# 0xPARC/plonkathon

Hardware: NVIDIA H100
Metric: plonk_proofs_per_s_2^20_gates (higher is better)
Workload: dtype u256 (BN254 Fr/Fq integers, 8x32-bit Montgomery limbs)

## Files before the change

plonkathon_b200/csrc/host_selftest.cpp:

```cpp
#include "field.cuh"
#include "curve.cuh"
#include "msm_digits.cuh"
#include "modinv.cuh"
#include "msm_bucket.cuh"
#include "msm_sort.cuh"
#include "ntt_shard.cuh"
#include <algorithm>
#include <vector>
#include <cstring>
using namespace pb200;

template <class F> static F ld(const uint32_t* p) { F r; memcpy(r.v, p, 32); return r; }
template <class F> static void st(uint32_t* p, const F& a) { memcpy(p, a.v, 32); }

extern "C" {
int hs_field_op(int field, int op, const uint32_t* a, const uint32_t* b, uint32_t* out) {
#define RUN(F)                                                   \
  {                                                              \
    F x = ld<F>(a), y = ld<F>(b), r;                             \
    switch (op) {                                                \
      case 0: r = fp_add(x, y); break;                           \
      case 1: r = fp_sub(x, y); break;                           \
      case 2: r = fp_mul(x, y); break;                           \
      case 3: r = fp_neg(x); break;                              \
// ... 190 lines not shown
  g.batch = batch;
  g.own_log = 0;
  g.own_rank = 0;
  if (hi >= 0xfffffff0u && hi != 0xffffffffu) {
    g.own_log = 0xffffffffu - hi;
    g.own_rank = lo;
    g.lo = 0;
    g.nloc = g.half >> g.own_log;
    if (!g.nloc || lo >= (1u << g.own_log)) return false;
  } else {
    if (hi > g.half) hi = g.half;
    if (lo >= hi) return false;
    g.lo = lo;
    g.nloc = hi - lo;
  }
  g.sets = fixed_base ? batch : g.W;
  g.nb = g.sets * g.nloc;
  return true;
}

static void host_scan(uint32_t* cnt, uint32_t len, uint32_t pad, uint32_t* off, uint32_t* max_out) {
  uint32_t run = 0, m = 0;
  for (uint32_t b = 0; b < len; b++) {
    off[b] = run;
    run += (cnt[b] + pad) & ~pad;
    m = std::max(m, cnt[b]);
    cnt[b] = 0;
  }
  off[len] = run;
  if (max_out) *max_out = m;
}

static void host_msm_sort(const MsmGeom& g, const std::vector<Fr>& sc, uint32_t n, uint32_t pad, uint32_t lb,
                          uint32_t T, uint32_t spb, uint32_t bin_nt, uint32_t chunk_nt, std::vector<uint32_t>& counts,
                          std::vector<uint32_t>& off, std::vector<uint32_t>& sorted) {
  const uint32_t nbins = ((g.nb - 1) >> lb) + 1;
  const uint32_t batch = g.fixed_base ? g.batch : 1;
  std::vector<uint32_t> bin_cnt(nbins, 0), bin_off(nbins + 1), chunk_first(nbins + 1);
  std::vector<SortEntry> binned((size_t)n * g.W * batch);
  counts.assign(g.nb + 1, 0);
  off.assign(g.nb + 1, 0);
  SortArgs a;
  for (uint32_t k = 0; k < 4; k++) a.sb.p[k] = k < batch ? sc.data() + (size_t)k * n : nullptr;
  a.n = n;
  a.from_mont = 0;
  a.g = g;
  a.lb = lb;
  a.nbins = nbins;
  a.T = T;
  a.bin_cnt = bin_cnt.data();
  a.bin_off = bin_off.data();
  a.binned = binned.data();
  a.chunk_first = chunk_first.data();
  a.counts = counts.data();
  a.offsets = off.data();
  a.sorted = nullptr;
  a.spb = spb;
  std::vector<uint32_t> sh_cnt(std::max(nbins, 1u << lb)), sh_loc(sh_cnt.size()), sh_base(sh_cnt.size()), runs;
  std::vector<SortEntry> bin_stage_buf((size_t)spb * g.W);
  std::vector<uint32_t> chunk_stage_buf(T);
  auto block_scan = [&](uint32_t len, uint32_t nt) {
    runs.assign(nt, 0);
    uint32_t run = 0;
    for (uint32_t t = 0; t < nt; t++) { runs[t] = run; run += scan_part_sum(sh_cnt.data(), len, t, nt); }
    return run;
  };
  const uint32_t bin_blocks = (n + spb - 1) / spb;
  for (uint32_t k = 0; k < batch; k++)
    for (uint32_t bx = 0; bx < bin_blocks; bx++) {
      for (uint32_t t = 0; t < bin_nt; t++) sort_zero(sh_cnt.data(), nbins, t, bin_nt);
      for (uint32_t t = 0; t < bin_nt; t++) bin_hist(a, bx, k, t, bin_nt, sh_cnt.data());
      for (uint32_t t = 0; t < bin_nt; t++) bin_flush(a, t, bin_nt, sh_cnt.data());
    }
  host_scan(bin_cnt.data(), nbins, 0, bin_off.data(), nullptr);
  for (uint32_t k = batch; k-- > 0;)
    for (uint32_t bx = bin_blocks; bx-- > 0;) {
      for (uint32_t t = 0; t < bin_nt; t++) sort_zero(sh_cnt.data(), nbins, t, bin_nt);
      for (uint32_t t = 0; t < bin_nt; t++) bin_hist(a, bx, k, t, bin_nt, sh_cnt.data());
      const uint32_t total = block_scan(nbins, bin_nt);
      for (uint32_t t = 0; t < bin_nt; t++)
        bin_reserve(a, t, bin_nt, runs[t], sh_cnt.data(), sh_loc.data(), sh_base.data());
      for (uint32_t t = 0; t < bin_nt; t++) bin_stage(a, bx, k, t, bin_nt, sh_cnt.data(), sh_loc.data(), bin_stage_buf.data());
      for (uint32_t t = 0; t < bin_nt; t++)
        bin_copy_out(a, t, bin_nt, total, sh_loc.data(), sh_base.data(), bin_stage_buf.data());
    }
  {
    std::vector<uint32_t> sums(256);
    for (uint32_t t = 0; t < 256; t++) sums[t] = chunk_map_sum(a, t);
    uint32_t run = 0;
    for (uint32_t t = 0; t < 256; t++) { const uint32_t s = sums[t]; sums[t] = run; run += s; }
    for (uint32_t t = 0; t < 256; t++) chunk_map_write(a, t, sums[t], run);
  }
  const uint32_t grid = 3;
  SortChunk ch;
  for (uint32_t bx = 0; bx < grid; bx++)
    for (uint32_t c = bx; chunk_locate(a, c, ch); c += grid) {
      for (uint32_t t = 0; t < chunk_nt; t++) sort_zero(sh_cnt.data(), ch.nkeys, t, chunk_nt);
      for (uint32_t t = 0; t < chunk_nt; t++) chunk_hist(a, ch, t, chunk_nt, sh_cnt.data());
      for (uint32_t t = 0; t < chunk_nt; t++) chunk_flush(a, ch, t, chunk_nt, sh_cnt.data());
    }
  host_scan(counts.data(), g.nb, pad, off.data(), &counts[g.nb]);
  sorted.assign(off[g.nb] + 2, PB_MSM_PAD);
  a.sorted = sorted.data();
  for (uint32_t bx = grid; bx-- > 0;)
    for (uint32_t c = bx; chunk_locate(a, c, ch); c += grid) {
      for (uint32_t t = 0; t < chunk_nt; t++) sort_zero(sh_cnt.data(), ch.nkeys, t, chunk_nt);
      for (uint32_t t = 0; t < chunk_nt; t++) chunk_hist(a, ch, t, chunk_nt, sh_cnt.data());
      const uint32_t total = block_scan(ch.nkeys, chunk_nt);
      for (uint32_t t = 0; t < chunk_nt; t++)
        chunk_reserve(a, ch, t, chunk_nt, runs[t], sh_cnt.data(), sh_loc.data(), sh_base.data());
      for (uint32_t t = 0; t < chunk_nt; t++) chunk_stage(a, ch, t, chunk_nt, sh_cnt.data(), sh_loc.data(), chunk_stage_buf.data());
      for (uint32_t t = 0; t < chunk_nt; t++)
        chunk_copy_out(a, ch, t, chunk_nt, sh_loc.data(), sh_base.data(), chunk_stage_buf.data());
      if (total != ch.hi - ch.lo) abort();
    }
}

extern "C" {
int hs_msm_sort(const uint32_t* scalars, uint32_t n, uint32_t batch, uint32_t c, int fixed_base, uint32_t lo,
                uint32_t hi, uint32_t pad, uint32_t lb, uint32_t T, uint32_t spb, uint32_t bin_nt, uint32_t chunk_nt,
                uint32_t* counts_out, uint32_t* off_out, uint32_t* sorted_out, uint32_t cap) {
  if (!n || !batch || batch > 4 || (!fixed_base && batch != 1) || c < 1 || c > 16 || !T || !bin_nt || !chunk_nt)
    return -1;
  MsmGeom g;
  if (!msm_geom(n, batch, c, fixed_base, lo, hi, g)) return -1;
  if (lb == 0xffffffffu) lb = sort_default_lb(g.nb);
  if (((g.nb - 1) >> lb) >= PB_SORT_MAX_BINS || (1u << lb) > PB_SORT_MAX_BIN_KEYS) return -1;
  if (!spb) spb = PB_SORT_BIN_STAGE / g.W;
  std::vector<Fr> sc((size_t)batch * n);
  for (size_t i = 0; i < sc.size(); i++) sc[i] = ld<Fr>(scalars + 8 * i);
  std::vector<uint32_t> counts, off, sorted;
  host_msm_sort(g, sc, n, pad ? 1 : 0, lb, T, spb, bin_nt, chunk_nt, counts, off, sorted);
  if (off[g.nb] > cap) return -1;
  memcpy(counts_out, counts.data(), counts.size() * 4);
  memcpy(off_out, off.data(), off.size() * 4);
  memcpy(sorted_out, sorted.data(), (size_t)off[g.nb] * 4);
  return (int)g.nb;
}

int hs_msm_pipeline(const uint32_t* points, uint32_t n, const uint32_t* scalars, uint32_t batch, uint32_t c,
                    int fixed_base, uint32_t lo, uint32_t hi, uint32_t B, uint32_t g0, uint32_t* out, uint8_t* out_inf) {
  if (!n || !batch || batch > 4 || (!fixed_base && batch != 1) || c < 1 || c > 16 || B < 2 || B > PB_AFF_BMAX) return -1;
  if (g0 < 2 || (g0 & (g0 - 1))) return -1;
  MsmGeom g;
  if (!msm_geom(n, batch, c, fixed_base, lo, hi, g)) return -1;
  std::vector<G1Affine> tab(fixed_base ? (size_t)g.W * n : n);
  for (uint32_t i = 0; i < n; i++) {
    tab[i].x = fp_to_mont(ld<Fq>(points + 16 * i));
    tab[i].y = fp_to_mont(ld<Fq>(points + 16 * i + 8));
  }
  if (fixed_base)
    for (uint32_t w = 1; w < g.W; w++)
      for (uint32_t i = 0; i < n; i++) {
        G1XYZZ a;
        g1_double_affine(a, tab[(size_t)(w - 1) * n + i]);
        for (uint32_t k = 1; k < c; k++) g1_double(a);
        g1_to_affine(a, tab[(size_t)w * n + i]);
      }
  std::vector<Fr> sc((size_t)batch * n);
  for (size_t i = 0; i < sc.size(); i++) sc[i] = ld<Fr>(scalars + 8 * i);
  std::vector<uint32_t> counts, off, sorted;
  host_msm_sort(g, sc, n, 1, sort_default_lb(g.nb), PB_SORT_CHUNK, PB_SORT_BIN_STAGE / g.W, PB_SORT_BIN_THREADS,
                PB_SORT_CHUNK_THREADS, counts, off, sorted);
  const uint32_t maxc = counts[g.nb];
  const uint64_t positions = (uint64_t)n * g.W * batch + g.nb, s_bound = positions / 2;
  std::vector<G1Affine> pts(s_bound + 1);
  AffAcc a;
  a.table = tab.data();
  a.sorted = sorted.data();
  a.pts = pts.data();
  a.off = off.data();
  a.cnt = counts.data();
  a.max_cnt = counts.data() + g.nb;
  a.nbl = g.nb;
  a.B = B;
  Fq pref[PB_AFF_BMAX];
  uint32_t desc[PB_AFF_BMAX];
  int rounds = 0;
  for (uint32_t r = 0; r < 32; r++) {
    a.r = r;
    if (r > 0 && maxc > (1u << r)) rounds = r + 1;
    if (r == 0) rounds = 1;
    const uint64_t T = aff_round_threads(s_bound, B, r) + 40;
    for (uint64_t t = T; t-- > 0;) {
      if (r == 0) aff_round0_thread(a, t, pref, desc);
      else aff_round_thread(a, t, pref, desc);
    }
  }
  ReduceArgs ra;
  ra.pts = pts.data(); ra.off = off.data(); ra.cnt = counts.data(); ra.xb = nullptr;
  ra.sets = g.sets; ra.m = g.nloc; ra.g = g0;
  std::vector<SR> cur((size_t)g.sets * reduce_groups(ra.m, ra.g)), nxt;
  ra.out = cur.data();
  for (uint64_t t = 0; t < cur.size() + 3; t++) reduce_level0_thread(ra, t);
  uint32_t m = reduce_groups(ra.m, ra.g), log_G = 0;
  while ((1u << log_G) < g0) log_G++;
// ... 72 lines not shown
```

plonkathon_b200/csrc/msm.cu:

```cuda
#include <algorithm>
#include <cstring>

#include "common.cuh"
#include "comm.cuh"
#include "msm_bucket.cuh"
#include "msm_digits.cuh"
#include "msm_sort.cuh"

namespace pb200 {

__device__ __forceinline__ G1Affine ld_affine(const G1Affine* p) {
  const uint4* q = reinterpret_cast<const uint4*>(p);
  uint4 a = __ldg(q), b = __ldg(q + 1), c = __ldg(q + 2), d = __ldg(q + 3);
  G1Affine r;
  r.x.v[0] = a.x; r.x.v[1] = a.y; r.x.v[2] = a.z; r.x.v[3] = a.w;
  r.x.v[4] = b.x; r.x.v[5] = b.y; r.x.v[6] = b.z; r.x.v[7] = b.w;
  r.y.v[0] = c.x; r.y.v[1] = c.y; r.y.v[2] = c.z; r.y.v[3] = c.w;
  r.y.v[4] = d.x; r.y.v[5] = d.y; r.y.v[6] = d.z; r.y.v[7] = d.w;
  return r;
}

__device__ __forceinline__ uint32_t block_exclusive_scan(uint32_t v, uint32_t* sh, uint32_t* total) {
  const uint32_t lane = threadIdx.x & 31, wid = threadIdx.x >> 5, nw = blockDim.x >> 5;
  uint32_t x = v;
  for (int d = 1; d < 32; d <<= 1) {
    uint32_t y = __shfl_up_sync(0xffffffffu, x, d);
    if ((int)lane >= d) x += y;
  }
  if (lane == 31) sh[wid] = x;
  __syncthreads();
  if (wid == 0) {
    uint32_t w = lane < nw ? sh[lane] : 0;
    for (int d = 1; d < 32; d <<= 1) {
      uint32_t y = __shfl_up_sync(0xffffffffu, w, d);
      if ((int)lane >= d) w += y;
    }
    if (lane < nw) sh[lane] = w;
  }
  __syncthreads();
  uint32_t base = wid ? sh[wid - 1] : 0;
  *total = sh[nw - 1];
  __syncthreads();
  return base + x - v;
}

__global__ void __launch_bounds__(PB_SORT_BIN_THREADS) k_msm_bin_count(SortArgs a) {
  __shared__ uint32_t sh_cnt[PB_SORT_MAX_BINS];
  const uint32_t t = threadIdx.x, nt = blockDim.x;
  sort_zero(sh_cnt, a.nbins, t, nt);
  __syncthreads();
  bin_hist(a, blockIdx.x, blockIdx.y, t, nt, sh_cnt);
  __syncthreads();
  bin_flush(a, t, nt, sh_cnt);
}

__global__ void __launch_bounds__(PB_SORT_BIN_THREADS) k_msm_bin_scatter(SortArgs a) {
  __shared__ uint32_t sh_cnt[PB_SORT_MAX_BINS], sh_loc[PB_SORT_MAX_BINS], sh_base[PB_SORT_MAX_BINS], sh_scan[32];
  extern __shared__ SortEntry stage[];
  const uint32_t t = threadIdx.x, nt = blockDim.x;
  sort_zero(sh_cnt, a.nbins, t, nt);
  __syncthreads();
  bin_hist(a, blockIdx.x, blockIdx.y, t, nt, sh_cnt);
  __syncthreads();
  uint32_t total;
  const uint32_t run = block_exclusive_scan(scan_part_sum(sh_cnt, a.nbins, t, nt), sh_scan, &total);
  bin_reserve(a, t, nt, run, sh_cnt, sh_loc, sh_base);
  __syncthreads();
  bin_stage(a, blockIdx.x, blockIdx.y, t, nt, sh_cnt, sh_loc, stage);
  __syncthreads();
  bin_copy_out(a, t, nt, total, sh_loc, sh_base, stage);
}

__global__ void __launch_bounds__(PB_SORT_CHUNK_THREADS) k_msm_chunk_count(SortArgs a) {
  __shared__ uint32_t sh_cnt[PB_SORT_MAX_BIN_KEYS];
  const uint32_t t = threadIdx.x, nt = blockDim.x;
  SortChunk ch;
  for (uint32_t c = blockIdx.x; chunk_locate(a, c, ch); c += gridDim.x) {
    sort_zero(sh_cnt, ch.nkeys, t, nt);
    __syncthreads();
    chunk_hist(a, ch, t, nt, sh_cnt);
    __syncthreads();
    chunk_flush(a, ch, t, nt, sh_cnt);
    __syncthreads();
  }
}

__global__ void __launch_bounds__(PB_SORT_CHUNK_THREADS) k_msm_chunk_place(SortArgs a) {
  __shared__ uint32_t sh_cnt[PB_SORT_MAX_BIN_KEYS], sh_loc[PB_SORT_MAX_BIN_KEYS], sh_base[PB_SORT_MAX_BIN_KEYS],
      sh_scan[32];
  extern __shared__ uint32_t stage_vals[];
  const uint32_t t = threadIdx.x, nt = blockDim.x;
  SortChunk ch;
  for (uint32_t c = blockIdx.x; chunk_locate(a, c, ch); c += gridDim.x) {
    sort_zero(sh_cnt, ch.nkeys, t, nt);
    __syncthreads();
    chunk_hist(a, ch, t, nt, sh_cnt);
    __syncthreads();
    uint32_t total;
    const uint32_t run = block_exclusive_scan(scan_part_sum(sh_cnt, ch.nkeys, t, nt), sh_scan, &total);
    chunk_reserve(a, ch, t, nt, run, sh_cnt, sh_loc, sh_base);
    __syncthreads();
    chunk_stage(a, ch, t, nt, sh_cnt, sh_loc, stage_vals);
    __syncthreads();
// ... 452 lines not shown
    }
  } else {
    comm = nullptr;
  }
  if (bucket_hi > g.half) bucket_hi = g.half;
  PB_CHECK(bucket_lo < bucket_hi, "empty MSM bucket range");
  g.lo = bucket_lo;
  g.nloc = bucket_hi - bucket_lo;
  g.sets = fixed_base ? batch : g.W;
  g.nb = g.sets * g.nloc;
  PB_CHECK((fixed_base ? (uint64_t)g.W * point_stride : n) < (1ull << 31), "MSM too large for 31-bit point ids");
  ScalarBatch sb;
  for (uint32_t k = 0; k < 4; k++) sb.p[k] = k < batch ? scalars[k] : nullptr;

  static const bool use_xyzz = [] { const char* e = getenv("PB200_MSM_ACC"); return !(e && !strcmp(e, "affine")); }();
  const uint32_t pad = use_xyzz ? 0 : 1;
  DevBuf& sorted = ctx->scratch[2];
  DevBuf& counts = ctx->scratch[3];
  DevBuf& offsets = ctx->scratch[4];
  DevBuf& lvl_a = ctx->scratch[6];
  DevBuf& lvl_b = ctx->scratch[7];
  const uint64_t entries = n * g.W * batch;
  const uint64_t positions = entries + (pad ? g.nb : 0);
  PB_CHECK(positions < (1ull << 30), "MSM too large (n * windows * batch must stay below 2^30)");
  sorted.ensure(positions * 4);
  counts.ensure((size_t)g.nb * 4 + 16);
  offsets.ensure((size_t)(g.nb + 1) * 4);
  uint32_t* max_cnt = counts.as<uint32_t>() + g.nb;
  const uint32_t n_tiles = (g.nb + PB_SCAN_TILE - 1) / PB_SCAN_TILE;
  PB_CHECK(n_tiles <= 8192, "too many buckets for the scan");
  ctx->msm_aff[1].ensure((size_t)8192 * 4);
  uint32_t* tile_sums = ctx->msm_aff[1].as<uint32_t>();

  const uint32_t lb = sort_default_lb(g.nb);
  PB_CHECK((1u << lb) <= PB_SORT_MAX_BIN_KEYS, "too many buckets for the sort");
  DevBuf& binned = ctx->scratch[8];
  DevBuf& bin_tab = ctx->scratch[9];
  binned.ensure(entries * sizeof(SortEntry));
  bin_tab.ensure((size_t)3 * (PB_SORT_MAX_BINS + 1) * 4);
  SortArgs sa;
  sa.sb = sb;
  sa.n = n;
  sa.from_mont = scalars_mont ? 1 : 0;
  sa.g = g;
  sa.lb = lb;
  sa.nbins = ((g.nb - 1) >> lb) + 1;
  sa.T = PB_SORT_CHUNK;
  uint32_t* bin_cnt = bin_tab.as<uint32_t>();
  uint32_t* bin_off = bin_cnt + PB_SORT_MAX_BINS + 1;
  sa.bin_cnt = bin_cnt;
  sa.bin_off = bin_off;
  sa.binned = binned.as<SortEntry>();
  sa.chunk_first = bin_off + PB_SORT_MAX_BINS + 1;
  sa.counts = counts.as<uint32_t>();
  sa.offsets = offsets.as<uint32_t>();
  sa.sorted = sorted.as<uint32_t>();
  sa.spb = PB_SORT_BIN_STAGE / g.W;
  const dim3 bin_grid((unsigned)((n + sa.spb - 1) / sa.spb), batch);
  const uint64_t chunk_bound = entries / PB_SORT_CHUNK + sa.nbins;
  const uint32_t count_grid = (uint32_t)std::min<uint64_t>((uint64_t)ctx->sm_count * 4, chunk_bound);
  const uint32_t place_grid = (uint32_t)std::min<uint64_t>((uint64_t)ctx->sm_count * 2, chunk_bound);
  const size_t bin_stage_bytes = PB_SORT_BIN_STAGE * sizeof(SortEntry), chunk_stage_bytes = PB_SORT_CHUNK * 4;
  PB_CUDA(cudaFuncSetAttribute(k_msm_bin_scatter, cudaFuncAttributeMaxDynamicSharedMemorySize, (int)bin_stage_bytes));
  PB_CUDA(cudaFuncSetAttribute(k_msm_chunk_place, cudaFuncAttributeMaxDynamicSharedMemorySize, (int)chunk_stage_bytes));

  cudaStream_t st = ctx->stream;
  ctx->time_begin(2);
  PB_CUDA(cudaMemsetAsync(counts.p, 0, (size_t)g.nb * 4 + 16, st));
  PB_CUDA(cudaMemsetAsync(bin_cnt, 0, (size_t)sa.nbins * 4, st));
  if (pad) PB_CUDA(cudaMemsetAsync(sorted.p, 0xff, positions * 4, st));
  k_msm_bin_count<<<bin_grid, PB_SORT_BIN_THREADS, 0, st>>>(sa);
  k_scan_tile_sums<<<1, 256, 0, st>>>(bin_cnt, sa.nbins, 0, tile_sums, nullptr);
  k_scan_tiles<<<1, 256, 0, st>>>(tile_sums, 1, bin_off + sa.nbins);
  k_scan_apply<<<1, 256, 0, st>>>(bin_cnt, sa.nbins, 0, tile_sums, bin_off);
  k_msm_bin_scatter<<<bin_grid, PB_SORT_BIN_THREADS, bin_stage_bytes, st>>>(sa);
  k_msm_chunk_map<<<1, 256, 0, st>>>(sa);
  k_msm_chunk_count<<<count_grid, PB_SORT_CHUNK_THREADS, 0, st>>>(sa);
  k_scan_tile_sums<<<n_tiles, 256, 0, st>>>(counts.as<uint32_t>(), g.nb, pad, tile_sums, max_cnt);
  k_scan_tiles<<<1, 256, 0, st>>>(tile_sums, n_tiles, offsets.as<uint32_t>() + g.nb);
  k_scan_apply<<<n_tiles, 256, 0, st>>>(counts.as<uint32_t>(), g.nb, pad, tile_sums, offsets.as<uint32_t>());
  k_msm_chunk_place<<<place_grid, PB_SORT_CHUNK_THREADS, chunk_stage_bytes, st>>>(sa);
  ctx->time_end(2);
  ctx->launches += 11;

  ReduceArgs ra;
  ra.pts = nullptr; ra.off = offsets.as<uint32_t>(); ra.cnt = counts.as<uint32_t>(); ra.xb = nullptr;
  if (!use_xyzz) {
    const uint64_t s_bound = positions / 2;
    DevBuf& pts = ctx->msm_aff[0];
    pts.ensure(s_bound * sizeof(G1Affine));
    AffAcc a;
    a.table = points;
    a.sorted = sorted.as<uint32_t>();
    a.pts = pts.as<G1Affine>();
    a.off = offsets.as<uint32_t>();
    a.cnt = counts.as<uint32_t>();
    a.max_cnt = max_cnt;
    a.nbl = g.nb;
    uint64_t cap = fixed_base ? n * g.W : n;
    uint32_t max_rounds = 1;
    while (max_rounds < 32 && (1ull << max_rounds) < cap) max_rounds++;
    ctx->time_begin(0);
    for (uint32_t r = 0; r < std::min<uint32_t>(max_rounds, PB_AFF_GRID_ROUNDS); r++) {
      a.r = r;
      a.B = pick_B(ctx, s_bound, r);
      const uint64_t threads = aff_round_threads(s_bound, a.B, r);
      if (r == 0) k_aff_round0<<<(unsigned)((threads + 127) / 128), 128, 0, st>>>(a);
      else k_aff_round<<<(unsigned)((threads + 127) / 128), 128, 0, st>>>(a);
      ctx->launches++;
    }
    if (max_rounds > PB_AFF_GRID_ROUNDS) {
      a.B = 32;
      k_aff_tail<<<1, 256, 0, st>>>(a, s_bound);
      ctx->launches++;
    }
    ctx->time_end(0);
// ... 311 lines not shown
```

plonkathon_b200/csrc/msm_sort.cuh:

```cuda
#pragma once
#include "msm_digits.cuh"

namespace pb200 {

#define PB_SORT_MAX_BINS 2048
#define PB_SORT_MAX_BIN_KEYS 2048
#define PB_SORT_BIN_THREADS 512
#define PB_SORT_BIN_STAGE 8192
#define PB_SORT_CHUNK_THREADS 512
#define PB_SORT_CHUNK 16384
static_assert(PB_SORT_MAX_BINS <= 256 * 8, "k_msm_chunk_map and the bin scan take one block of 256 x 8 bins");

struct alignas(8) SortEntry {
  uint32_t key, val;
};

struct SortArgs {
  ScalarBatch sb;
  uint64_t n;
  int from_mont;
  MsmGeom g;
  uint32_t spb;
  uint32_t lb;
  uint32_t nbins;
  uint32_t T;
  uint32_t* bin_cnt;
  const uint32_t* bin_off;
  SortEntry* binned;
  uint32_t* chunk_first;
  uint32_t* counts;
  const uint32_t* offsets;
  uint32_t* sorted;
};

PB_HD uint32_t sort_default_lb(uint32_t nb) {
  uint32_t lb = 0;
  while (((nb - 1) >> lb) >= PB_SORT_MAX_BINS) lb++;
  return lb;
}

PB_HD uint32_t sort_add(uint32_t* p, uint32_t v) {
#if defined(__CUDA_ARCH__)
  return atomicAdd(p, v);
#else
  const uint32_t o = *p;
  *p = o + v;
  return o;
#endif
}

PB_HD void sort_zero(uint32_t* sh, uint32_t len, uint32_t t, uint32_t nt) {
  for (uint32_t b = t; b < len; b += nt) sh[b] = 0;
}

PB_HD uint32_t scan_part_sum(const uint32_t* sh, uint32_t len, uint32_t t, uint32_t nt) {
  const uint32_t per = (len + nt - 1) / nt;
  uint32_t s = 0;
  for (uint32_t b = t * per; b < t * per + per && b < len; b++) s += sh[b];
  return s;
}

template <class F>
PB_HD void sort_walk(const SortArgs& a, uint32_t bx, uint32_t k, uint32_t t, uint32_t nt, F f) {
  const uint64_t end = (uint64_t)(bx + 1) * a.spb < a.n ? (uint64_t)(bx + 1) * a.spb : a.n;
  for (uint64_t i = (uint64_t)bx * a.spb + t; i < end; i += nt) {
    DigitWalk dw(a.sb.p[k], i, a.from_mont);
    for (uint32_t w = 0; w < a.g.W; w++) {
      uint32_t neg, d = dw.next(w, a.g, neg);
      if (!d) continue;
      const uint32_t key = msm_bucket_key(a.g, k, w, d);
      if (key != 0xffffffffu) f(key, (uint32_t)((uint64_t)w * a.g.point_stride + i) | (neg << 31));
    }
  }
}

PB_HD void bin_hist(const SortArgs& a, uint32_t bx, uint32_t k, uint32_t t, uint32_t nt, uint32_t* sh_cnt) {
  sort_walk(a, bx, k, t, nt, [&](uint32_t key, uint32_t) { sort_add(&sh_cnt[key >> a.lb], 1u); });
}

PB_HD void bin_flush(const SortArgs& a, uint32_t t, uint32_t nt, const uint32_t* sh_cnt) {
  for (uint32_t b = t; b < a.nbins; b += nt)
    if (sh_cnt[b]) sort_add(&a.bin_cnt[b], sh_cnt[b]);
}

PB_HD void bin_reserve(const SortArgs& a, uint32_t t, uint32_t nt, uint32_t run, uint32_t* sh_cnt, uint32_t* sh_loc,
                       uint32_t* sh_base) {
  const uint32_t per = (a.nbins + nt - 1) / nt;
  for (uint32_t b = t * per; b < t * per + per && b < a.nbins; b++) {
    const uint32_t c = sh_cnt[b];
    sh_loc[b] = run;
    run += c;
    if (c) sh_base[b] = a.bin_off[b] + sort_add(&a.bin_cnt[b], c);
    sh_cnt[b] = 0;
  }
}

PB_HD void bin_stage(const SortArgs& a, uint32_t bx, uint32_t k, uint32_t t, uint32_t nt, uint32_t* sh_cnt,
                     const uint32_t* sh_loc, SortEntry* stage) {
  sort_walk(a, bx, k, t, nt, [&](uint32_t key, uint32_t val) {
    const uint32_t b = key >> a.lb;
    SortEntry e;
    e.key = key;
    e.val = val;
    stage[sh_loc[b] + sort_add(&sh_cnt[b], 1u)] = e;
  });
}

PB_HD void bin_copy_out(const SortArgs& a, uint32_t t, uint32_t nt, uint32_t total, const uint32_t* sh_loc,
                        const uint32_t* sh_base, const SortEntry* stage) {
  for (uint32_t p = t; p < total; p += nt) {
    const SortEntry e = stage[p];
    const uint32_t b = e.key >> a.lb;
    a.binned[sh_base[b] + p - sh_loc[b]] = e;
  }
}

PB_HD uint32_t chunk_map_sum(const SortArgs& a, uint32_t t) {
  uint32_t s = 0;
  for (uint32_t b = 8 * t; b < 8 * t + 8 && b < a.nbins; b++) s += (a.bin_cnt[b] + a.T - 1) / a.T;
  return s;
}
PB_HD void chunk_map_write(const SortArgs& a, uint32_t t, uint32_t run, uint32_t total) {
  for (uint32_t b = 8 * t; b < 8 * t + 8 && b < a.nbins; b++) {
    a.chunk_first[b] = run;
    run += (a.bin_cnt[b] + a.T - 1) / a.T;
  }
  if (t == 0) a.chunk_first[a.nbins] = total;
}

struct SortChunk {
  uint32_t lo, hi;
  uint32_t key0, nkeys;
};

PB_HD bool chunk_locate(const SortArgs& a, uint32_t c, SortChunk& ch) {
  if (c >= a.chunk_first[a.nbins]) return false;
  uint32_t l = 0, h = a.nbins;
  while (l < h) {
    const uint32_t m = (l + h) >> 1;
    if (a.chunk_first[m] > c) h = m; else l = m + 1;
  }
  const uint32_t b = l - 1;
  ch.lo = a.bin_off[b] + (c - a.chunk_first[b]) * a.T;
  ch.hi = a.bin_off[b + 1] - ch.lo > a.T ? ch.lo + a.T : a.bin_off[b + 1];
  ch.key0 = b << a.lb;
  ch.nkeys = a.g.nb - ch.key0 < (1u << a.lb) ? a.g.nb - ch.key0 : 1u << a.lb;
  return true;
}

PB_HD void chunk_hist(const SortArgs& a, const SortChunk& ch, uint32_t t, uint32_t nt, uint32_t* sh_cnt) {
  for (uint32_t i = ch.lo + t; i < ch.hi; i += nt) sort_add(&sh_cnt[a.binned[i].key - ch.key0], 1u);
}

PB_HD void chunk_flush(const SortArgs& a, const SortChunk& ch, uint32_t t, uint32_t nt, const uint32_t* sh_cnt) {
  for (uint32_t l = t; l < ch.nkeys; l += nt)
    if (sh_cnt[l]) sort_add(&a.counts[ch.key0 + l], sh_cnt[l]);
}

PB_HD void chunk_reserve(const SortArgs& a, const SortChunk& ch, uint32_t t, uint32_t nt, uint32_t run,
                         uint32_t* sh_cnt, uint32_t* sh_loc, uint32_t* sh_base) {
// ... 33 lines not shown
```

Before: 24.60.

## Add single-pass per-bin placement sort for MSM buckets with heavy-bin fallback

Adds a k_msm_bin_place kernel that, for bins small enough to fit in shared memory, counts, scans and scatters entries within one block, writing counts, offsets and sorted output directly. Bins above the cap take the old chunked path, with a new per-bin heavy scan replacing the global bucket-count scan when no padding is needed. Bin histograms are also limited to a per-batch window, bin-scan tiling is widened to multiple blocks, and the bin-width heuristic now targets the placement stage size. The aim is to remove the separate global count/scan/place passes and the large memsets. The cost is more code paths and a dependence on how the scalar distribution spreads across bins.

```diff
diff --git a/plonkathon_b200/csrc/host_selftest.cpp b/plonkathon_b200/csrc/host_selftest.cpp
--- a/plonkathon_b200/csrc/host_selftest.cpp
+++ b/plonkathon_b200/csrc/host_selftest.cpp
@@ -246,14 +246,18 @@
 }
 
 static void host_msm_sort(const MsmGeom& g, const std::vector<Fr>& sc, uint32_t n, uint32_t pad, uint32_t lb,
-                          uint32_t T, uint32_t spb, uint32_t bin_nt, uint32_t chunk_nt, std::vector<uint32_t>& counts,
-                          std::vector<uint32_t>& off, std::vector<uint32_t>& sorted) {
+                          uint32_t T, uint32_t spb, uint32_t bin_nt, uint32_t chunk_nt, uint32_t cap, uint32_t place_nt,
+                          std::vector<uint32_t>& counts, std::vector<uint32_t>& off, std::vector<uint32_t>& sorted,
+                          uint32_t* heavy = nullptr) {
   const uint32_t nbins = ((g.nb - 1) >> lb) + 1;
   const uint32_t batch = g.fixed_base ? g.batch : 1;
+  if (pad) cap = 0;
   std::vector<uint32_t> bin_cnt(nbins, 0), bin_off(nbins + 1), chunk_first(nbins + 1);
   std::vector<SortEntry> binned((size_t)n * g.W * batch);
-  counts.assign(g.nb + 1, 0);
-  off.assign(g.nb + 1, 0);
+  counts.assign(g.nb + 1, pad ? 0 : 0xdeadbeefu);
+  counts[g.nb] = 0;
+  off.assign(g.nb + 1, 0xdeadbeefu);
+  sorted.assign((size_t)n * g.W * batch + g.nb + 2, PB_MSM_PAD);
   SortArgs a;
   for (uint32_t k = 0; k < 4; k++) a.sb.p[k] = k < batch ? sc.data() + (size_t)k * n : nullptr;
   a.n = n;
@@ -262,42 +266,73 @@
   a.lb = lb;
   a.nbins = nbins;
   a.T = T;
+  a.cap = cap;
   a.bin_cnt = bin_cnt.data();
   a.bin_off = bin_off.data();
   a.binned = binned.data();
   a.chunk_first = chunk_first.data();
   a.counts = counts.data();
   a.offsets = off.data();
-  a.sorted = nullptr;
+  a.sorted = sorted.data();
   a.spb = spb;
   std::vector<uint32_t> sh_cnt(std::max(nbins, 1u << lb)), sh_loc(sh_cnt.size()), sh_base(sh_cnt.size()), runs;
   std::vector<SortEntry> bin_stage_buf((size_t)spb * g.W);
-  std::vector<uint32_t> chunk_stage_buf(T);
-  auto block_scan = [&](uint32_t len, uint32_t nt) {
+  std::vector<uint32_t> chunk_stage_buf(T), place_stage_buf(std::max(cap, 1u));
+  std::vector<uint32_t> kr((size_t)place_nt * PB_SORT_PLACE_PER), val(kr.size());
+  auto block_scan_of = [&](uint32_t nt, auto part) {
     runs.assign(nt, 0);
     uint32_t run = 0;
-    for (uint32_t t = 0; t < nt; t++) { runs[t] = run; run += scan_part_sum(sh_cnt.data(), len, t, nt); }
+    for (uint32_t t = 0; t < nt; t++) { runs[t] = run; run += part(t); }
     return run;
+  };
+  auto block_scan = [&](uint32_t len, uint32_t nt) {
+    return block_scan_of(nt, [&](uint32_t t) { return scan_part_sum(sh_cnt.data(), len, t, nt); });
   };
   const uint32_t bin_blocks = (n + spb - 1) / spb;
   for (uint32_t k = 0; k < batch; k++)
     for (uint32_t bx = 0; bx < bin_blocks; bx++) {
-      for (uint32_t t = 0; t < bin_nt; t++) sort_zero(sh_cnt.data(), nbins, t, bin_nt);
+      const uint32_t len = sort_window(g, lb, k).len;
+      for (uint32_t t = 0; t < bin_nt; t++) sort_zero(sh_cnt.data(), len, t, bin_nt);
       for (uint32_t t = 0; t < bin_nt; t++) bin_hist(a, bx, k, t, bin_nt, sh_cnt.data());
-      for (uint32_t t = 0; t < bin_nt; t++) bin_flush(a, t, bin_nt, sh_cnt.data());
+      for (uint32_t t = 0; t < bin_nt; t++) bin_flush(a, k, t, bin_nt, sh_cnt.data());
     }
   host_scan(bin_cnt.data(), nbins, 0, bin_off.data(), nullptr);
   for (uint32_t k = batch; k-- > 0;)
     for (uint32_t bx = bin_blocks; bx-- > 0;) {
-      for (uint32_t t = 0; t < bin_nt; t++) sort_zero(sh_cnt.data(), nbins, t, bin_nt);
+      const uint32_t len = sort_window(g, lb, k).len;
+      for (uint32_t t = 0; t < bin_nt; t++) sort_zero(sh_cnt.data(), len, t, bin_nt);
       for (uint32_t t = 0; t < bin_nt; t++) bin_hist(a, bx, k, t, bin_nt, sh_cnt.data());
-      const uint32_t total = block_scan(nbins, bin_nt);
+      const uint32_t total = block_scan(len, bin_nt);
       for (uint32_t t = 0; t < bin_nt; t++)
-        bin_reserve(a, t, bin_nt, runs[t], sh_cnt.data(), sh_loc.data(), sh_base.data());
+        bin_reserve(a, k, t, bin_nt, runs[t], sh_cnt.data(), sh_loc.data(), sh_base.data());
       for (uint32_t t = 0; t < bin_nt; t++) bin_stage(a, bx, k, t, bin_nt, sh_cnt.data(), sh_loc.data(), bin_stage_buf.data());
       for (uint32_t t = 0; t < bin_nt; t++)
-        bin_copy_out(a, t, bin_nt, total, sh_loc.data(), sh_base.data(), bin_stage_buf.data());
-    }
+        bin_copy_out(a, k, t, bin_nt, total, sh_loc.data(), sh_base.data(), bin_stage_buf.data());
+    }
+  if (!pad) {
+    if (heavy) *heavy = 0;
+    for (uint32_t b = nbins; b-- > 0;) {
+      const SortBin sb = sort_bin(a, b);
+      bool take = true;
+      for (uint32_t t = 0; t < place_nt; t++) take = place_begin(a, sb, b, t, place_nt);
+      if (!take) {
+        if (heavy) ++*heavy;
+        continue;
+      }
+      for (uint32_t t = 0; t < place_nt; t++) sort_zero(sh_cnt.data(), sb.nkeys, t, place_nt);
+      for (uint32_t t = 0; t < place_nt; t++)
+        place_load(a, sb, t, place_nt, sh_cnt.data(), kr.data() + t * PB_SORT_PLACE_PER, val.data() + t * PB_SORT_PLACE_PER);
+      const uint32_t total = block_scan(sb.nkeys, place_nt);
+      if (total != sb.hi - sb.lo) abort();
+      uint32_t m = 0;
+      for (uint32_t t = 0; t < place_nt; t++) m = std::max(m, place_offsets(a, sb, t, place_nt, runs[t], sh_cnt.data()));
+      for (uint32_t t = 0; t < place_nt; t++)
+        place_stage(sb, t, place_nt, sh_cnt.data(), kr.data() + t * PB_SORT_PLACE_PER, val.data() + t * PB_SORT_PLACE_PER,
+                    place_stage_buf.data());
+      counts[g.nb] = std::max(counts[g.nb], m);
+      for (uint32_t t = 0; t < place_nt; t++) place_copy_out(a, sb, t, place_nt, place_stage_buf.data());
+    }
+  }
   {
     std::vector<uint32_t> sums(256);
     for (uint32_t t = 0; t < 256; t++) sums[t] = chunk_map_sum(a, t);
@@ -313,9 +348,17 @@
       for (uint32_t t = 0; t < chunk_nt; t++) chunk_hist(a, ch, t, chunk_nt, sh_cnt.data());
       for (uint32_t t = 0; t < chunk_nt; t++) chunk_flush(a, ch, t, chunk_nt, sh_cnt.data());
     }
-  host_scan(counts.data(), g.nb, pad, off.data(), &counts[g.nb]);
-  sorted.assign(off[g.nb] + 2, PB_MSM_PAD);
-  a.sorted = sorted.data();
+  if (pad) {
+    host_scan(counts.data(), g.nb, pad, off.data(), &counts[g.nb]);
+  } else {
+    for (uint32_t b = 0; b < nbins; b++) {
+      if (bin_cnt[b] <= cap) continue;
+      const SortBin sb = sort_bin(a, b);
+      const uint32_t nt = 256;
+      block_scan_of(nt, [&](uint32_t t) { return heavy_scan_sum(a, sb, t, nt); });
+      for (uint32_t t = 0; t < nt; t++) counts[g.nb] = std::max(counts[g.nb], heavy_scan_write(a, sb, t, nt, runs[t]));
+    }
+  }
   for (uint32_t bx = grid; bx-- > 0;)
     for (uint32_t c = bx; chunk_locate(a, c, ch); c += grid) {
       for (uint32_t t = 0; t < chunk_nt; t++) sort_zero(sh_cnt.data(), ch.nkeys, t, chunk_nt);
@@ -328,28 +371,40 @@
         chunk_copy_out(a, ch, t, chunk_nt, sh_loc.data(), sh_base.data(), chunk_stage_buf.data());
       if (total != ch.hi - ch.lo) abort();
     }
+  sorted.resize((size_t)off[g.nb] + 2);
 }
 
 extern "C" {
-int hs_msm_sort(const uint32_t* scalars, uint32_t n, uint32_t batch, uint32_t c, int fixed_base, uint32_t lo,
-                uint32_t hi, uint32_t pad, uint32_t lb, uint32_t T, uint32_t spb, uint32_t bin_nt, uint32_t chunk_nt,
-                uint32_t* counts_out, uint32_t* off_out, uint32_t* sorted_out, uint32_t cap) {
-  if (!n || !batch || batch > 4 || (!fixed_base && batch != 1) || c < 1 || c > 16 || !T || !bin_nt || !chunk_nt)
+int hs_msm_sort_place(const uint32_t* scalars, uint32_t n, uint32_t batch, uint32_t c, int fixed_base, uint32_t lo,
+                      uint32_t hi, uint32_t pad, uint32_t lb, uint32_t T, uint32_t spb, uint32_t bin_nt,
+                      uint32_t chunk_nt, uint32_t place_nt, uint32_t cap, uint32_t* counts_out, uint32_t* off_out,
+                      uint32_t* sorted_out, uint32_t room, uint32_t* heavy) {
+  if (!n || !batch || batch > 4 || (!fixed_base && batch != 1) || c < 1 || c > 16 || !T || !bin_nt || !chunk_nt ||
+      !place_nt || cap > place_nt * PB_SORT_PLACE_PER || cap > PB_SORT_PLACE_STAGE)
     return -1;
   MsmGeom g;
   if (!msm_geom(n, batch, c, fixed_base, lo, hi, g)) return -1;
-  if (lb == 0xffffffffu) lb = sort_default_lb(g.nb);
-  if (((g.nb - 1) >> lb) >= PB_SORT_MAX_BINS || (1u << lb) > PB_SORT_MAX_BIN_KEYS) return -1;
+  if (lb == 0xffffffffu) lb = sort_default_lb(g, n);
+  if (!sort_lb_fits(g, lb)) return -1;
   if (!spb) spb = PB_SORT_BIN_STAGE / g.W;
   std::vector<Fr> sc((size_t)batch * n);
   for (size_t i = 0; i < sc.size(); i++) sc[i] = ld<Fr>(scalars + 8 * i);
   std::vector<uint32_t> counts, off, sorted;
-  host_msm_sort(g, sc, n, pad ? 1 : 0, lb, T, spb, bin_nt, chunk_nt, counts, off, sorted);
-  if (off[g.nb] > cap) return -1;
+  *heavy = 0;
+  host_msm_sort(g, sc, n, pad ? 1 : 0, lb, T, spb, bin_nt, chunk_nt, cap, place_nt, counts, off, sorted, heavy);
+  if (off[g.nb] > room) return -1;
   memcpy(counts_out, counts.data(), counts.size() * 4);
   memcpy(off_out, off.data(), off.size() * 4);
   memcpy(sorted_out, sorted.data(), (size_t)off[g.nb] * 4);
   return (int)g.nb;
+}
+
+int hs_msm_sort(const uint32_t* scalars, uint32_t n, uint32_t batch, uint32_t c, int fixed_base, uint32_t lo,
+                uint32_t hi, uint32_t pad, uint32_t lb, uint32_t T, uint32_t spb, uint32_t bin_nt, uint32_t chunk_nt,
+                uint32_t* counts_out, uint32_t* off_out, uint32_t* sorted_out, uint32_t cap) {
+  uint32_t heavy;
+  return hs_msm_sort_place(scalars, n, batch, c, fixed_base, lo, hi, pad, lb, T, spb, bin_nt, chunk_nt,
+                           PB_SORT_PLACE_THREADS, PB_SORT_PLACE_STAGE, counts_out, off_out, sorted_out, cap, &heavy);
 }
 
 int hs_msm_pipeline(const uint32_t* points, uint32_t n, const uint32_t* scalars, uint32_t batch, uint32_t c,
@@ -374,8 +429,8 @@
   std::vector<Fr> sc((size_t)batch * n);
   for (size_t i = 0; i < sc.size(); i++) sc[i] = ld<Fr>(scalars + 8 * i);
   std::vector<uint32_t> counts, off, sorted;
-  host_msm_sort(g, sc, n, 1, sort_default_lb(g.nb), PB_SORT_CHUNK, PB_SORT_BIN_STAGE / g.W, PB_SORT_BIN_THREADS,
-                PB_SORT_CHUNK_THREADS, counts, off, sorted);
+  host_msm_sort(g, sc, n, 1, sort_default_lb(g, n), PB_SORT_CHUNK, PB_SORT_BIN_STAGE / g.W, PB_SORT_BIN_THREADS,
+                PB_SORT_CHUNK_THREADS, 0, PB_SORT_PLACE_THREADS, counts, off, sorted);
   const uint32_t maxc = counts[g.nb];
   const uint64_t positions = (uint64_t)n * g.W * batch + g.nb, s_bound = positions / 2;
   std::vector<G1Affine> pts(s_bound + 1);
diff --git a/plonkathon_b200/csrc/msm.cu b/plonkathon_b200/csrc/msm.cu
--- a/plonkathon_b200/csrc/msm.cu
+++ b/plonkathon_b200/csrc/msm.cu
@@ -45,30 +45,71 @@
 }
 
 __global__ void __launch_bounds__(PB_SORT_BIN_THREADS) k_msm_bin_count(SortArgs a) {
-  __shared__ uint32_t sh_cnt[PB_SORT_MAX_BINS];
+  __shared__ uint32_t sh_cnt[PB_SORT_BIN_WINDOW];
   const uint32_t t = threadIdx.x, nt = blockDim.x;
-  sort_zero(sh_cnt, a.nbins, t, nt);
+  sort_zero(sh_cnt, sort_window(a.g, a.lb, blockIdx.y).len, t, nt);
   __syncthreads();
   bin_hist(a, blockIdx.x, blockIdx.y, t, nt, sh_cnt);
   __syncthreads();
-  bin_flush(a, t, nt, sh_cnt);
+  bin_flush(a, blockIdx.y, t, nt, sh_cnt);
 }
 
 __global__ void __launch_bounds__(PB_SORT_BIN_THREADS) k_msm_bin_scatter(SortArgs a) {
-  __shared__ uint32_t sh_cnt[PB_SORT_MAX_BINS], sh_loc[PB_SORT_MAX_BINS], sh_base[PB_SORT_MAX_BINS], sh_scan[32];
+  __shared__ uint32_t sh_cnt[PB_SORT_BIN_WINDOW], sh_loc[PB_SORT_BIN_WINDOW], sh_base[PB_SORT_BIN_WINDOW], sh_scan[32];
   extern __shared__ SortEntry stage[];
+  const uint32_t t = threadIdx.x, nt = blockDim.x, len = sort_window(a.g, a.lb, blockIdx.y).len;
+  sort_zero(sh_cnt, len, t, nt);
+  __syncthreads();
+  bin_hist(a, blockIdx.x, blockIdx.y, t, nt, sh_cnt);
+  __syncthreads();
+  uint32_t total;
+  const uint32_t run = block_exclusive_scan(scan_part_sum(sh_cnt, len, t, nt), sh_scan, &total);
+  bin_reserve(a, blockIdx.y, t, nt, run, sh_cnt, sh_loc, sh_base);
+  __syncthreads();
+  bin_stage(a, blockIdx.x, blockIdx.y, t, nt, sh_cnt, sh_loc, stage);
+  __syncthreads();
+  bin_copy_out(a, blockIdx.y, t, nt, total, sh_loc, sh_base, stage);
+}
+
+__device__ __forceinline__ void block_max_to(uint32_t m, uint32_t* sh, uint32_t* out) {
+  for (int d = 16; d > 0; d >>= 1) m = max(m, __shfl_xor_sync(0xffffffffu, m, d));
+  if ((threadIdx.x & 31) == 0) sh[threadIdx.x >> 5] = m;
+  __syncthreads();
+  if (threadIdx.x < 32) {
+    m = threadIdx.x < (blockDim.x >> 5) ? sh[threadIdx.x] : 0;
+    for (int d = 16; d > 0; d >>= 1) m = max(m, __shfl_xor_sync(0xffffffffu, m, d));
+    if (threadIdx.x == 0 && m) atomicMax(out, m);
+  }
+}
+
+__global__ void __launch_bounds__(PB_SORT_PLACE_THREADS, 2) k_msm_bin_place(SortArgs a) {
+  __shared__ uint32_t sh_cnt[PB_SORT_MAX_BIN_KEYS], sh_scan[32];
+  extern __shared__ uint32_t stage_vals[];
   const uint32_t t = threadIdx.x, nt = blockDim.x;
-  sort_zero(sh_cnt, a.nbins, t, nt);
-  __syncthreads();
-  bin_hist(a, blockIdx.x, blockIdx.y, t, nt, sh_cnt);
+  const SortBin sb = sort_bin(a, blockIdx.x);
+  if (!place_begin(a, sb, blockIdx.x, t, nt)) return;
+  uint32_t kr[PB_SORT_PLACE_PER], val[PB_SORT_PLACE_PER];
+  sort_zero(sh_cnt, sb.nkeys, t, nt);
+  __syncthreads();
+  place_load(a, sb, t, nt, sh_cnt, kr, val);
   __syncthreads();
   uint32_t total;
-  const uint32_t run = block_exclusive_scan(scan_part_sum(sh_cnt, a.nbins, t, nt), sh_scan, &total);
-  bin_reserve(a, t, nt, run, sh_cnt, sh_loc, sh_base);
-  __syncthreads();
-  bin_stage(a, blockIdx.x, blockIdx.y, t, nt, sh_cnt, sh_loc, stage);
-  __syncthreads();
-  bin_copy_out(a, t, nt, total, sh_loc, sh_base, stage);
+  const uint32_t run = block_exclusive_scan(scan_part_sum(sh_cnt, sb.nkeys, t, nt), sh_scan, &total);
+  const uint32_t m = place_offsets(a, sb, t, nt, run, sh_cnt);
+  __syncthreads();
+  place_stage(sb, t, nt, sh_cnt, kr, val, stage_vals);
+  block_max_to(m, sh_scan, a.counts + a.g.nb);
+  place_copy_out(a, sb, t, nt, stage_vals);
+}
+
+__global__ void __launch_bounds__(256) k_msm_heavy_scan(SortArgs a) {
+  __shared__ uint32_t sh[32];
+  if (a.bin_cnt[blockIdx.x] <= a.cap) return;
+  const uint32_t t = threadIdx.x, nt = blockDim.x;
+  const SortBin sb = sort_bin(a, blockIdx.x);
+  uint32_t total;
+  const uint32_t run = block_exclusive_scan(heavy_scan_sum(a, sb, t, nt), sh, &total);
+  block_max_to(heavy_scan_write(a, sb, t, nt, run), sh, a.counts + a.g.nb);
 }
 
 __global__ void __launch_bounds__(PB_SORT_CHUNK_THREADS) k_msm_chunk_count(SortArgs a) {
@@ -587,8 +628,8 @@
   ctx->msm_aff[1].ensure((size_t)8192 * 4);
   uint32_t* tile_sums = ctx->msm_aff[1].as<uint32_t>();
 
-  const uint32_t lb = sort_default_lb(g.nb);
-  PB_CHECK((1u << lb) <= PB_SORT_MAX_BIN_KEYS, "too many buckets for the sort");
+  const uint32_t lb = sort_default_lb(g, n);
+  PB_CHECK(lb != 0xffffffffu, "too many buckets for the sort");
   DevBuf& binned = ctx->scratch[8];
   DevBuf& bin_tab = ctx->scratch[9];
   binned.ensure(entries * sizeof(SortEntry));
@@ -601,6 +642,7 @@
   sa.lb = lb;
   sa.nbins = ((g.nb - 1) >> lb) + 1;
   sa.T = PB_SORT_CHUNK;
+  sa.cap = pad ? 0 : PB_SORT_PLACE_STAGE;
   uint32_t* bin_cnt = bin_tab.as<uint32_t>();
   uint32_t* bin_off = bin_cnt + PB_SORT_MAX_BINS + 1;
   sa.bin_cnt = bin_cnt;
@@ -612,31 +654,38 @@
   sa.sorted = sorted.as<uint32_t>();
   sa.spb = PB_SORT_BIN_STAGE / g.W;
   const dim3 bin_grid((unsigned)((n + sa.spb - 1) / sa.spb), batch);
+  const uint32_t bin_tiles = (sa.nbins + PB_SCAN_TILE - 1) / PB_SCAN_TILE;
   const uint64_t chunk_bound = entries / PB_SORT_CHUNK + sa.nbins;
   const uint32_t count_grid = (uint32_t)std::min<uint64_t>((uint64_t)ctx->sm_count * 4, chunk_bound);
   const uint32_t place_grid = (uint32_t)std::min<uint64_t>((uint64_t)ctx->sm_count * 2, chunk_bound);
   const size_t bin_stage_bytes = PB_SORT_BIN_STAGE * sizeof(SortEntry), chunk_stage_bytes = PB_SORT_CHUNK * 4;
+  const size_t place_stage_bytes = PB_SORT_PLACE_STAGE * 4;
   PB_CUDA(cudaFuncSetAttribute(k_msm_bin_scatter, cudaFuncAttributeMaxDynamicSharedMemorySize, (int)bin_stage_bytes));
   PB_CUDA(cudaFuncSetAttribute(k_msm_chunk_place, cudaFuncAttributeMaxDynamicSharedMemorySize, (int)chunk_stage_bytes));
 
   cudaStream_t st = ctx->stream;
   ctx->time_begin(2);
-  PB_CUDA(cudaMemsetAsync(counts.p, 0, (size_t)g.nb * 4 + 16, st));
+  PB_CUDA(cudaMemsetAsync(pad ? counts.p : (void*)max_cnt, 0, pad ? (size_t)g.nb * 4 + 16 : 16, st));
   PB_CUDA(cudaMemsetAsync(bin_cnt, 0, (size_t)sa.nbins * 4, st));
   if (pad) PB_CUDA(cudaMemsetAsync(sorted.p, 0xff, positions * 4, st));
   k_msm_bin_count<<<bin_grid, PB_SORT_BIN_THREADS, 0, st>>>(sa);
-  k_scan_tile_sums<<<1, 256, 0, st>>>(bin_cnt, sa.nbins, 0, tile_sums, nullptr);
-  k_scan_tiles<<<1, 256, 0, st>>>(tile_sums, 1, bin_off + sa.nbins);
-  k_scan_apply<<<1, 256, 0, st>>>(bin_cnt, sa.nbins, 0, tile_sums, bin_off);
+  k_scan_tile_sums<<<bin_tiles, 256, 0, st>>>(bin_cnt, sa.nbins, 0, tile_sums, nullptr);
+  k_scan_tiles<<<1, 256, 0, st>>>(tile_sums, bin_tiles, bin_off + sa.nbins);
+  k_scan_apply<<<bin_tiles, 256, 0, st>>>(bin_cnt, sa.nbins, 0, tile_sums, bin_off);
   k_msm_bin_scatter<<<bin_grid, PB_SORT_BIN_THREADS, bin_stage_bytes, st>>>(sa);
+  if (!pad) k_msm_bin_place<<<sa.nbins, PB_SORT_PLACE_THREADS, place_stage_bytes, st>>>(sa);
   k_msm_chunk_map<<<1, 256, 0, st>>>(sa);
   k_msm_chunk_count<<<count_grid, PB_SORT_CHUNK_THREADS, 0, st>>>(sa);
-  k_scan_tile_sums<<<n_tiles, 256, 0, st>>>(counts.as<uint32_t>(), g.nb, pad, tile_sums, max_cnt);
-  k_scan_tiles<<<1, 256, 0, st>>>(tile_sums, n_tiles, offsets.as<uint32_t>() + g.nb);
-  k_scan_apply<<<n_tiles, 256, 0, st>>>(counts.as<uint32_t>(), g.nb, pad, tile_sums, offsets.as<uint32_t>());
+  if (pad) {
+    k_scan_tile_sums<<<n_tiles, 256, 0, st>>>(counts.as<uint32_t>(), g.nb, pad, tile_sums, max_cnt);
+    k_scan_tiles<<<1, 256, 0, st>>>(tile_sums, n_tiles, offsets.as<uint32_t>() + g.nb);
+    k_scan_apply<<<n_tiles, 256, 0, st>>>(counts.as<uint32_t>(), g.nb, pad, tile_sums, offsets.as<uint32_t>());
+  } else {
+    k_msm_heavy_scan<<<sa.nbins, 256, 0, st>>>(sa);
+  }
   k_msm_chunk_place<<<place_grid, PB_SORT_CHUNK_THREADS, chunk_stage_bytes, st>>>(sa);
   ctx->time_end(2);
-  ctx->launches += 11;
+  ctx->launches += pad ? 11 : 9;
 
   ReduceArgs ra;
   ra.pts = nullptr; ra.off = offsets.as<uint32_t>(); ra.cnt = counts.as<uint32_t>(); ra.xb = nullptr;
diff --git a/plonkathon_b200/csrc/msm_sort.cuh b/plonkathon_b200/csrc/msm_sort.cuh
--- a/plonkathon_b200/csrc/msm_sort.cuh
+++ b/plonkathon_b200/csrc/msm_sort.cuh
@@ -3,13 +3,18 @@
 
 namespace pb200 {
 
-#define PB_SORT_MAX_BINS 2048
+#define PB_SORT_MAX_BINS 8192
+#define PB_SORT_BIN_WINDOW 2048
 #define PB_SORT_MAX_BIN_KEYS 2048
 #define PB_SORT_BIN_THREADS 512
 #define PB_SORT_BIN_STAGE 8192
+#define PB_SORT_PLACE_THREADS 512
+#define PB_SORT_PLACE_PER 16
+#define PB_SORT_PLACE_STAGE (PB_SORT_PLACE_THREADS * PB_SORT_PLACE_PER)
 #define PB_SORT_CHUNK_THREADS 512
 #define PB_SORT_CHUNK 16384
-static_assert(PB_SORT_MAX_BINS <= 256 * 8, "k_msm_chunk_map and the bin scan take one block of 256 x 8 bins");
+static_assert(PB_SORT_MAX_BINS <= 256 * 32, "k_msm_chunk_map takes one block of 256 threads x 32 bins");
+static_assert(PB_SORT_PLACE_STAGE <= 65536 && PB_SORT_MAX_BIN_KEYS <= 65536, "k_msm_bin_place packs key | rank << 16");
 
 struct alignas(8) SortEntry {
   uint32_t key, val;
@@ -24,18 +29,47 @@
   uint32_t lb;
   uint32_t nbins;
   uint32_t T;
+  uint32_t cap;
   uint32_t* bin_cnt;
   const uint32_t* bin_off;
   SortEntry* binned;
   uint32_t* chunk_first;
   uint32_t* counts;
-  const uint32_t* offsets;
+  uint32_t* offsets;
   uint32_t* sorted;
 };
 
-PB_HD uint32_t sort_default_lb(uint32_t nb) {
-  uint32_t lb = 0;
-  while (((nb - 1) >> lb) >= PB_SORT_MAX_BINS) lb++;
+struct SortWindow {
+  uint32_t b0, len;
+};
+PB_HD SortWindow sort_window(const MsmGeom& g, uint32_t lb, uint32_t k) {
+  SortWindow w;
+  if (g.fixed_base) {
+    w.b0 = (k * g.nloc) >> lb;
+    w.len = (((k + 1) * g.nloc - 1) >> lb) - w.b0 + 1;
+  } else {
+    w.b0 = 0;
+    w.len = ((g.nb - 1) >> lb) + 1;
+  }
+  return w;
+}
+
+PB_HD bool sort_lb_fits(const MsmGeom& g, uint32_t lb) {
+  if (lb > 31 || (1u << lb) > PB_SORT_MAX_BIN_KEYS || ((g.nb - 1) >> lb) >= PB_SORT_MAX_BINS) return false;
+  for (uint32_t k = 0; k < (g.fixed_base ? g.batch : 1); k++)
+    if (sort_window(g, lb, k).len > PB_SORT_BIN_WINDOW) return false;
+  return true;
+}
+
+PB_HD uint32_t sort_default_lb(const MsmGeom& g, uint64_t n) {
+  uint32_t lo = 0;
+  while (lo <= 11 && !sort_lb_fits(g, lo)) lo++;
+  if (lo > 11) return 0xffffffffu;
+  const uint64_t per_key_x_half = g.fixed_base ? n * g.W : n;
+  uint32_t lb = lo;
+  while (lb < 11 && sort_lb_fits(g, lb + 1) &&
+         (per_key_x_half << (lb + 1)) <= (uint64_t)PB_SORT_PLACE_STAGE / 8 * 7 * g.half)
+    lb++;
   return lb;
 }
 
@@ -75,30 +109,34 @@
 }
 
 PB_HD void bin_hist(const SortArgs& a, uint32_t bx, uint32_t k, uint32_t t, uint32_t nt, uint32_t* sh_cnt) {
-  sort_walk(a, bx, k, t, nt, [&](uint32_t key, uint32_t) { sort_add(&sh_cnt[key >> a.lb], 1u); });
-}
-
-PB_HD void bin_flush(const SortArgs& a, uint32_t t, uint32_t nt, const uint32_t* sh_cnt) {
-  for (uint32_t b = t; b < a.nbins; b += nt)
-    if (sh_cnt[b]) sort_add(&a.bin_cnt[b], sh_cnt[b]);
-}
-
-PB_HD void bin_reserve(const SortArgs& a, uint32_t t, uint32_t nt, uint32_t run, uint32_t* sh_cnt, uint32_t* sh_loc,
-                       uint32_t* sh_base) {
-  const uint32_t per = (a.nbins + nt - 1) / nt;
-  for (uint32_t b = t * per; b < t * per + per && b < a.nbins; b++) {
+  const uint32_t b0 = sort_window(a.g, a.lb, k).b0;
+  sort_walk(a, bx, k, t, nt, [&](uint32_t key, uint32_t) { sort_add(&sh_cnt[(key >> a.lb) - b0], 1u); });
+}
+
+PB_HD void bin_flush(const SortArgs& a, uint32_t k, uint32_t t, uint32_t nt, const uint32_t* sh_cnt) {
+  const SortWindow w = sort_window(a.g, a.lb, k);
+  for (uint32_t b = t; b < w.len; b += nt)
+    if (sh_cnt[b]) sort_add(&a.bin_cnt[w.b0 + b], sh_cnt[b]);
+}
+
+PB_HD void bin_reserve(const SortArgs& a, uint32_t k, uint32_t t, uint32_t nt, uint32_t run, uint32_t* sh_cnt,
+                       uint32_t* sh_loc, uint32_t* sh_base) {
+  const SortWindow w = sort_window(a.g, a.lb, k);
+  const uint32_t per = (w.len + nt - 1) / nt;
+  for (uint32_t b = t * per; b < t * per + per && b < w.len; b++) {
     const uint32_t c = sh_cnt[b];
     sh_loc[b] = run;
     run += c;
-    if (c) sh_base[b] = a.bin_off[b] + sort_add(&a.bin_cnt[b], c);
+    if (c) sh_base[b] = a.bin_off[w.b0 + b] + sort_add(&a.bin_cnt[w.b0 + b], c);
     sh_cnt[b] = 0;
   }
 }
 
 PB_HD void bin_stage(const SortArgs& a, uint32_t bx, uint32_t k, uint32_t t, uint32_t nt, uint32_t* sh_cnt,
                      const uint32_t* sh_loc, SortEntry* stage) {
+  const uint32_t b0 = sort_window(a.g, a.lb, k).b0;
   sort_walk(a, bx, k, t, nt, [&](uint32_t key, uint32_t val) {
-    const uint32_t b = key >> a.lb;
+    const uint32_t b = (key >> a.lb) - b0;
     SortEntry e;
     e.key = key;
     e.val = val;
@@ -106,26 +144,114 @@
   });
 }
 
-PB_HD void bin_copy_out(const SortArgs& a, uint32_t t, uint32_t nt, uint32_t total, const uint32_t* sh_loc,
+PB_HD void bin_copy_out(const SortArgs& a, uint32_t k, uint32_t t, uint32_t nt, uint32_t total, const uint32_t* sh_loc,
                         const uint32_t* sh_base, const SortEntry* stage) {
+  const uint32_t b0 = sort_window(a.g, a.lb, k).b0;
   for (uint32_t p = t; p < total; p += nt) {
     const SortEntry e = stage[p];
-    const uint32_t b = e.key >> a.lb;
+    const uint32_t b = (e.key >> a.lb) - b0;
     a.binned[sh_base[b] + p - sh_loc[b]] = e;
   }
 }
 
+struct SortBin {
+  uint32_t lo, hi;
+  uint32_t key0, nkeys;
+};
+
+PB_HD SortBin sort_bin(const SortArgs& a, uint32_t b) {
+  SortBin sb;
+  sb.lo = a.bin_off[b];
+  sb.hi = a.bin_off[b + 1];
+  sb.key0 = b << a.lb;
+  sb.nkeys = a.g.nb - sb.key0 < (1u << a.lb) ? a.g.nb - sb.key0 : 1u << a.lb;
+  return sb;
+}
+
+PB_HD bool place_begin(const SortArgs& a, const SortBin& sb, uint32_t b, uint32_t t, uint32_t nt) {
+  if (b == 0 && t == 0) a.offsets[a.g.nb] = a.bin_off[a.nbins];
+  if (sb.hi - sb.lo <= a.cap) return true;
+  for (uint32_t l = t; l < sb.nkeys; l += nt) a.counts[sb.key0 + l] = 0;
+  return false;
+}
+
+PB_HD void place_load(const SortArgs& a, const SortBin& sb, uint32_t t, uint32_t nt, uint32_t* sh_cnt, uint32_t* kr,
+                      uint32_t* val) {
+#if defined(__CUDA_ARCH__)
+#pragma unroll
+#endif
+  for (uint32_t j = 0; j < PB_SORT_PLACE_PER; j++) {
+    const uint32_t i = sb.lo + j * nt + t;
+    if (i < sb.hi) {
+      const SortEntry e = a.binned[i];
+      const uint32_t l = e.key - sb.key0;
+      kr[j] = l | sort_add(&sh_cnt[l], 1u) << 16;
+      val[j] = e.val;
+    }
+  }
+}
+
+PB_HD uint32_t place_offsets(const SortArgs& a, const SortBin& sb, uint32_t t, uint32_t nt, uint32_t run,
+                             uint32_t* sh_cnt) {
+  const uint32_t per = (sb.nkeys + nt - 1) / nt;
+  uint32_t m = 0;
+  for (uint32_t l = t * per; l < t * per + per && l < sb.nkeys; l++) {
+    const uint32_t c = sh_cnt[l];
+    a.counts[sb.key0 + l] = c;
+    a.offsets[sb.key0 + l] = sb.lo + run;
+    sh_cnt[l] = run;
+    run += c;
+    m = c > m ? c : m;
+  }
+  return m;
+}
+
+PB_HD void place_stage(const SortBin& sb, uint32_t t, uint32_t nt, const uint32_t* sh_cnt, const uint32_t* kr,
+                       const uint32_t* val, uint32_t* stage) {
+#if defined(__CUDA_ARCH__)
+#pragma unroll
+#endif
+  for (uint32_t j = 0; j < PB_SORT_PLACE_PER; j++)
+    if (sb.lo + j * nt + t < sb.hi) stage[sh_cnt[kr[j] & 0xffffu] + (kr[j] >> 16)] = val[j];
+}
+
+PB_HD void place_copy_out(const SortArgs& a, const SortBin& sb, uint32_t t, uint32_t nt, const uint32_t* stage) {
+  for (uint32_t p = t; p < sb.hi - sb.lo; p += nt) a.sorted[sb.lo + p] = stage[p];
+}
+
+PB_HD uint32_t chunk_count_of(const SortArgs& a, uint32_t b) {
+  const uint32_t c = a.bin_cnt[b];
+  return c > a.cap ? (c + a.T - 1) / a.T : 0;
+}
 PB_HD uint32_t chunk_map_sum(const SortArgs& a, uint32_t t) {
+  const uint32_t per = (a.nbins + 255) / 256;
   uint32_t s = 0;
-  for (uint32_t b = 8 * t; b < 8 * t + 8 && b < a.nbins; b++) s += (a.bin_cnt[b] + a.T - 1) / a.T;
+  for (uint32_t b = per * t; b < per * t + per && b < a.nbins; b++) s += chunk_count_of(a, b);
   return s;
 }
 PB_HD void chunk_map_write(const SortArgs& a, uint32_t t, uint32_t run, uint32_t total) {
-  for (uint32_t b = 8 * t; b < 8 * t + 8 && b < a.nbins; b++) {
+  const uint32_t per = (a.nbins + 255) / 256;
+  for (uint32_t b = per * t; b < per * t + per && b < a.nbins; b++) {
     a.chunk_first[b] = run;
-    run += (a.bin_cnt[b] + a.T - 1) / a.T;
+    run += chunk_count_of(a, b);
   }
   if (t == 0) a.chunk_first[a.nbins] = total;
+}
+
+PB_HD uint32_t heavy_scan_sum(const SortArgs& a, const SortBin& sb, uint32_t t, uint32_t nt) {
+  return scan_part_sum(a.counts + sb.key0, sb.nkeys, t, nt);
+}
+PB_HD uint32_t heavy_scan_write(const SortArgs& a, const SortBin& sb, uint32_t t, uint32_t nt, uint32_t run) {
+  const uint32_t per = (sb.nkeys + nt - 1) / nt;
+  uint32_t m = 0;
+  for (uint32_t l = t * per; l < t * per + per && l < sb.nkeys; l++) {
+    const uint32_t c = a.counts[sb.key0 + l];
+    a.offsets[sb.key0 + l] = sb.lo + run;
+    a.counts[sb.key0 + l] = 0;
+    run += c;
+    m = c > m ? c : m;
+  }
+  return m;
 }
 
 struct SortChunk {
```

New measurement: 25.20 (median of 6 runs). +2.4%, better.
